# sgl-project/rbg

Hardware: AMD Instinct MI355X
Metric: output tok/s (llama-3-8b P/D-disagg serving, KV migration over xGMI) (higher is better)
Workload: dtype bf16; 1 GPU; model=llama-3-8b, global_batch=128, seq_len=2048, parallelism=pd1 (1 prefill + 1 decode, prefill colocated with decode0)

## Files before the change

rbg_amd/models/llama.py:

```python
from __future__ import annotations

import math
from dataclasses import dataclass
from typing import Optional

import torch
import torch.nn as nn

from .. import ops
from ..engine.config import ModelConfig
from ..engine.kv_cache import PagedKVCache


@dataclass
class ForwardBatch:
    mode: str
    positions: torch.Tensor
    slot_mapping: torch.Tensor
    cu_seqlens: Optional[torch.Tensor] = None
    cu_seqlens_k: Optional[torch.Tensor] = None
    kv_gather_slots: Optional[torch.Tensor] = None
    block_tables: Optional[torch.Tensor] = None
    context_lens: Optional[torch.Tensor] = None
    decode_num_splits: int = 0
# ... 100 lines not shown
        wk = _linear_weight(full_kv, cfg.hidden_size, device, dtype, gen,
                            shard_dim=0, tp_size=tp.size, tp_rank=tp.rank)
        wv = _linear_weight(full_kv, cfg.hidden_size, device, dtype, gen,
                            shard_dim=0, tp_size=tp.size, tp_rank=tp.rank)
        self.wqkv = nn.Parameter(torch.cat([wq, wk, wv], dim=0),
                                 requires_grad=False)
        self.wo = _linear_weight(cfg.hidden_size, full_q, device, dtype, gen,
                                 shard_dim=1, tp_size=tp.size,
                                 tp_rank=tp.rank)
        self.q_out, self.kv_out = q_out, kv_out
        self.q_norm = self.k_norm = None
        if cfg.qk_norm:
            self.q_norm = nn.Parameter(torch.ones(cfg.head_dim, device=device,
                                                  dtype=dtype),
                                       requires_grad=False)
            self.k_norm = nn.Parameter(torch.ones(cfg.head_dim, device=device,
                                                  dtype=dtype),
                                       requires_grad=False)

    def forward(self, x: torch.Tensor, batch: ForwardBatch,
                kv: PagedKVCache, cos_sin: torch.Tensor,
                add_norm=None) -> torch.Tensor:
        T = x.shape[0]
        qkv = ops.linear(x, self.wqkv)
        q = qkv[:, :self.q_out]
        k = qkv[:, self.q_out:self.q_out + self.kv_out]
        v = qkv[:, self.q_out + self.kv_out:]
        if self.q_norm is not None:
            q = ops.rmsnorm(q.contiguous().view(-1, self.head_dim),
                            self.q_norm,
                            self.cfg.rms_eps).view(T, self.q_out)
            k = ops.rmsnorm(k.contiguous().view(-1, self.head_dim),
                            self.k_norm,
                            self.cfg.rms_eps).view(T, self.kv_out)
            v = v.clone(memory_format=torch.contiguous_format)
        key_cache = kv.key_cache(self.layer_idx)
        value_cache = kv.value_cache(self.layer_idx)
        fp8 = kv.fp8
        if fp8:
            ops.rope_store_kv(q, k, v, key_cache, value_cache, cos_sin,
                              batch.positions, batch.slot_mapping,
                              kv.k_scale_log2, kv.v_scale_log2)
        else:
            ops.rope_store_kv(q, k, v, key_cache, value_cache, cos_sin,
                              batch.positions, batch.slot_mapping)
        q3 = q.view(T, self.heads, self.head_dim)
        if batch.mode == "prefill":
            if fp8:
                if batch.kv_gather_slots is None:
                    raise RuntimeError("an fp8 KV pool prefills through the "
                                       "gather path: kv_gather_slots unset")
                k_full = ops.kv_gather_dequant(
                    key_cache, batch.kv_gather_slots, kv.k_scale_log2)
                v_full = ops.kv_gather_dequant(
                    value_cache, batch.kv_gather_slots, kv.v_scale_log2)
                o = ops.prefill_attention(q3, k_full, v_full,
                                          batch.cu_seqlens, self.scale,
                                          batch.cu_seqlens_k)
            elif batch.kv_gather_slots is not None:
                ps = key_cache.shape[2]
                slots = batch.kv_gather_slots.long()
                pages, offs = slots // ps, slots % ps
# ... 190 lines not shown
```

rbg_amd/ops/__init__.py:

```python
from __future__ import annotations

import os

import torch

from . import reference

_hip = None
_hip_err: Exception | None = None
try:
    from . import _hip_ops as _hip
except Exception as e:
    _hip_err = e

HAVE_HIP = _hip is not None


def _check_stale() -> None:
    import hashlib
    here = os.path.dirname(os.path.abspath(__file__))
    stamp = os.path.join(here, "_hip_ops.srchash")
    if not os.path.exists(stamp):
        return
    h = hashlib.sha256()
# ... 26 lines not shown
    return _hip


def _on_gpu(t: torch.Tensor) -> bool:
    return t.is_cuda


SKINNY_GEMM = int(os.environ.get("RBG_SKINNY_GEMM", "1"))


def linear(x: torch.Tensor, w: torch.Tensor) -> torch.Tensor:
    if _use_skinny_gemm(x, w):
        return _require_hip().skinny_gemm(
            x if x.is_contiguous() else x.contiguous(), w)
    return torch.nn.functional.linear(x, w)


def _use_skinny_gemm(x: torch.Tensor, w: torch.Tensor) -> bool:
    return bool(SKINNY_GEMM and _on_gpu(x) and x.dim() == 2 and
                x.dtype == torch.bfloat16 and 1 <= x.shape[0] <= 128 and
                w.shape[0] % 32 == 0 and x.shape[1] % 512 == 0 and
                (w.shape[0] <= 4608 or
                 (x.shape[0] <= 64 and w.shape[0] <= 8192)))


def linear_add_rmsnorm(x: torch.Tensor, w: torch.Tensor,
                       residual: torch.Tensor, norm_weight: torch.Tensor,
                       eps: float) -> torch.Tensor:
    if _use_skinny_gemm(x, w):
        return _require_hip().skinny_gemm_add_rmsnorm(
            x if x.is_contiguous() else x.contiguous(), w, residual,
            norm_weight, eps)
    h = linear(x, w)
    fused_add_rmsnorm(h, residual, norm_weight, eps)
    return h


def rmsnorm(x: torch.Tensor, weight: torch.Tensor, eps: float) -> torch.Tensor:
    if _on_gpu(x):
        return _require_hip().rmsnorm(x, weight, eps)
    return reference.rmsnorm(x, weight, eps)


def fused_add_rmsnorm(x: torch.Tensor, residual: torch.Tensor,
                      weight: torch.Tensor, eps: float) -> None:
    if _on_gpu(x):
# ... 144 lines not shown
```

rbg_amd/ops/hip/bindings.cpp:

```cpp
#include <torch/extension.h>
#include <ATen/hip/HIPContext.h>

#include <hip/hip_runtime.h>

#include <algorithm>
#include <cmath>
#include <cstring>
#include <vector>

extern "C" {
void launch_rmsnorm(void*, void*, const void*, float, int, int, hipStream_t);
void launch_fused_add_rmsnorm(void*, void*, const void*, float, int, int,
                              hipStream_t);
void launch_silu_mul(void*, const void*, int, int, hipStream_t);
void launch_rope_store_kv(void*, void*, const void*, void*, void*,
                          const void*, const void*, const void*, int, int,
                          int, int, int, int, int, hipStream_t);
void launch_decode_attention(void*, void*, void*, const void*, const void*,
                             const void*, const void*, const void*, float,
                             int, int, int, int, int, int, int, int, int,
                             hipStream_t);
void launch_prefill_attention(void*, const void*, const void*, const void*,
                              const void*, const void*, float, int, int, int,
                              int, int, int, hipStream_t);
void launch_mfma_probe(void*, const void*, const void*, int, int, hipStream_t);
void launch_mfma_probe32(void*, const void*, const void*, int, int, int,
                         hipStream_t);
void launch_skinny_gemm(void*, void*, const void*, const void*, int, int,
                        int, int, hipStream_t);
void launch_skinny_gemm_wide(void*, void*, const void*, const void*, int, int,
                             int, int, hipStream_t);
void launch_reduce_splits(void*, const void*, int, long, hipStream_t);
void launch_fold_add_rmsnorm(void*, const void*, void*, const void*, float,
                             int, int, int, hipStream_t);
void launch_kv_peer_copy(void*, const void*, const void*, const void*, int,
                         int, int, long, long, long, long, hipStream_t);
void launch_xgmi_allreduce(void*, const void*, void**, void**, int, int,
                           long, hipStream_t);
void launch_sample(void*, void*, const void*, const void*, const void*,
                   const void*, const void*, const void*, const void*, int,
                   int, hipStream_t);
void launch_rope_store_kv_fp8(void*, void*, const void*, void*, void*,
                              const void*, const void*, const void*, int, int,
                              int, int, int, int, float, float, hipStream_t);
void launch_kv_gather_dequant(void*, const void*, const void*, long, int, int,
                              int, float, hipStream_t);
void launch_decode_attention_fp8(void*, void*, void*, const void*, const void*,
                                 const void*, const void*, const void*, float,
                                 float, int, int, int, int, int, int, int,
                                 hipStream_t);
long xgmi_allreduce_signal_bytes();
long xgmi_allreduce_error_offset();
long xgmi_allreduce_counter_offset();
}
// ... 79 lines not shown
  out_sizes.back() = inter;
  auto out = torch::empty(out_sizes, x.options());
  if (tokens == 0) return out;
  launch_silu_mul(out.data_ptr(), x.data_ptr(), tokens, inter,
                  current_stream());
  return out;
}

static void check_bf16_rowslice(const torch::Tensor& t, const char* name) {
  TORCH_CHECK(t.is_cuda(), name, " must be on GPU");
  TORCH_CHECK(t.scalar_type() == torch::kBFloat16, name, " must be bf16");
  if (t.dim() == 2) {
    TORCH_CHECK(t.stride(1) == 1, name, " rows must be contiguous");
  } else {
    TORCH_CHECK(t.dim() == 3 && t.stride(2) == 1 &&
                t.stride(1) == t.size(2), name,
                " must be [T, H, D] with contiguous (H, D) rows");
  }
}

void rope_store_kv(torch::Tensor q, torch::Tensor k, torch::Tensor v,
                   torch::Tensor key_cache, torch::Tensor value_cache,
                   torch::Tensor cos_sin, torch::Tensor positions,
                   torch::Tensor slot_mapping) {
  check_bf16_rowslice(q, "q");
  check_bf16_rowslice(k, "k");
  check_bf16_rowslice(v, "v");
  TORCH_CHECK(k.stride(0) == v.stride(0), "k/v stride mismatch");
  TORCH_CHECK(cos_sin.scalar_type() == torch::kFloat32, "cos_sin fp32");
  TORCH_CHECK(positions.scalar_type() == torch::kInt32, "positions int32");
  TORCH_CHECK(slot_mapping.scalar_type() == torch::kInt32, "slots int32");
  check_kv_caches(key_cache, value_cache);
  check_i32_gpu(positions, "positions");
  check_i32_gpu(slot_mapping, "slot_mapping");
  TORCH_CHECK(cos_sin.is_cuda() && cos_sin.is_contiguous() &&
              cos_sin.dim() == 2, "cos_sin must be a contiguous 2-D GPU tensor");
  const int tokens = q.size(0);
  const int head_dim = key_cache.size(3);
  const int num_kv_heads = key_cache.size(1);
  const int page_size = key_cache.size(2);
  TORCH_CHECK(cos_sin.size(1) == head_dim,
              "cos_sin row width must equal the cache head_dim");
  TORCH_CHECK(k.size(0) == tokens && v.size(0) == tokens &&
              positions.numel() == tokens && slot_mapping.numel() == tokens,
              "q/k/v/positions/slot_mapping token counts differ");
  const int64_t q_width = q.numel() / std::max(tokens, 1);
  const int64_t k_width = k.numel() / std::max(tokens, 1);
  const int64_t v_width = v.numel() / std::max(tokens, 1);
  TORCH_CHECK(k_width == (int64_t)num_kv_heads * head_dim && v_width == k_width,
              "k/v rows must be cache KVH * head_dim wide");
  TORCH_CHECK(q_width % head_dim == 0,
              "q row width must be a multiple of the cache head_dim");
  if (tokens == 0) return;
  const int num_q_heads = (int)(q_width / head_dim);
  launch_rope_store_kv(q.data_ptr(), k.data_ptr(), v.data_ptr(),
                       key_cache.data_ptr(), value_cache.data_ptr(),
                       cos_sin.data_ptr(), positions.data_ptr(),
                       slot_mapping.data_ptr(), tokens, num_q_heads,
                       num_kv_heads, head_dim, page_size,
                       (int)q.stride(0), (int)k.stride(0),
                       current_stream());
}

bool pick_in_wg_combine(int64_t combine, int64_t num_splits, bool mfma_pair,
                        const char* what) {
  TORCH_CHECK(combine >= 0 && combine <= 2,
              "combine must be 0 (auto), 1 (kernel) or 2 (in-workgroup)");
  const bool can = mfma_pair && (num_splits == 2 || num_splits == 4);
  TORCH_CHECK(combine != 2 || can, "combine = 2 needs ", what,
              ", a page size of 16 and 2 or 4 splits");
  const bool in_wg = combine != 1 && can;
  TORCH_CHECK(!in_wg || num_splits == 2 || num_splits == 4,
              "in-workgroup combine with ", num_splits, " splits");
  return in_wg;
}

torch::Tensor decode_attention(torch::Tensor q, torch::Tensor key_cache,
                               torch::Tensor value_cache,
                               torch::Tensor block_tables,
                               torch::Tensor context_lens, double scale,
                               int64_t num_splits, int64_t variant,
                               int64_t combine = 0) {
  TORCH_CHECK(q.is_cuda() && q.scalar_type() == torch::kBFloat16 &&
              q.dim() == 3 && q.stride(2) == 1 &&
// ... 240 lines not shown
  return d;
}

}

static int pick_gemm_splits(int N, int K) {
  const int n_groups = N >> 5;
  for (int s : {8, 4, 2})
    if (n_groups * s <= 512 && n_groups * s >= 192 && K % (s * 256) == 0)
      return s;
  for (int s : {4, 2})
    if (n_groups * s >= 128 && K % (s * 256) == 0) return s;
  return 1;
}

bool skinny_gemm_supported(int64_t M, int64_t N, int64_t K) {
  return M >= 1 && M <= 256 && (N % 32) == 0 && (K % 256) == 0;
}

bool skinny_gemm_wide_supported(int64_t M, int64_t N) {
  return M >= 1 && M <= 128 && (N % 64) == 0;
}

static int pick_gemm_panel(int64_t M, int64_t N) {
  return M > 32 && skinny_gemm_wide_supported(M, N) ? 64 : 32;
}

namespace {

int skinny_gemm_launch(const torch::Tensor& a, const torch::Tensor& w,
                       int64_t force_splits, int64_t panel, torch::Tensor& c,
                       torch::Tensor& ws) {
  check_bf16_contig(a, "a");
  check_bf16_contig(w, "w");
  TORCH_CHECK(a.dim() == 2 && w.dim() == 2, "a and w must be 2-D");
  TORCH_CHECK(a.device() == w.device(), "a/w device mismatch");
  const int64_t M = a.size(0), K = a.size(1), N = w.size(0);
  TORCH_CHECK(w.size(1) == K, "K mismatch");
  TORCH_CHECK(skinny_gemm_supported(M, N, K), "unsupported skinny shape");
  TORCH_CHECK(force_splits == 0 || force_splits == 1 || force_splits == 2 ||
                  force_splits == 4 || force_splits == 8,
              "force_splits must be 0 (auto), 1, 2, 4 or 8");
  TORCH_CHECK(force_splits == 0 || K % (force_splits * 256) == 0,
              "K must be a multiple of force_splits * 256");
  TORCH_CHECK(panel == 0 || panel == 32 || panel == 64,
              "panel must be 0 (auto), 32 or 64");
  TORCH_CHECK(panel != 64 || skinny_gemm_wide_supported(M, N),
              "panel 64 needs M <= 128 and N % 64 == 0");
  const int splits = force_splits > 0 ? (int)force_splits
                                      : pick_gemm_splits((int)N, (int)K);
  if (panel == 0) panel = pick_gemm_panel(M, N);
  void* cp = nullptr;
  void* wsp = nullptr;
  if (splits > 1) {
    ws = torch::empty({splits, M, N}, a.options().dtype(torch::kFloat32));
    wsp = ws.data_ptr();
  } else {
    c = torch::empty({M, N}, a.options());
    cp = c.data_ptr();
  }
  (panel == 64 ? launch_skinny_gemm_wide : launch_skinny_gemm)(
      cp, wsp, a.data_ptr(), w.data_ptr(), (int)M, (int)N, (int)K, splits,
      current_stream());
  return splits;
}

}

torch::Tensor skinny_gemm(torch::Tensor a, torch::Tensor w,
                          int64_t force_splits = 0, int64_t panel = 0) {
  torch::Tensor c, ws;
  const int splits = skinny_gemm_launch(a, w, force_splits, panel, c, ws);
  if (splits > 1) {
    c = torch::empty({a.size(0), w.size(0)}, a.options());
    launch_reduce_splits(c.data_ptr(), ws.data_ptr(), splits,
                         (long)c.numel(), current_stream());
  }
  return c;
}

torch::Tensor skinny_gemm_add_rmsnorm(torch::Tensor a, torch::Tensor w,
                                      torch::Tensor residual,
                                      torch::Tensor norm_weight, double eps,
                                      int64_t force_splits = 0,
                                      int64_t panel = 0) {
  check_bf16_contig(residual, "residual");
  check_bf16_contig(norm_weight, "norm_weight");
  TORCH_CHECK(a.dim() == 2 && w.dim() == 2, "a and w must be 2-D");
  TORCH_CHECK(residual.dim() == 2 && residual.size(0) == a.size(0) &&
                  residual.size(1) == w.size(0),
              "residual must be [M, N]");
  TORCH_CHECK(norm_weight.numel() == w.size(0),
              "norm_weight must have N elements");
  TORCH_CHECK(residual.device() == a.device() &&
                  norm_weight.device() == a.device(),
              "a/residual/norm_weight device mismatch");
  torch::Tensor c, ws;
  const int splits = skinny_gemm_launch(a, w, force_splits, panel, c, ws);
  const int M = (int)a.size(0), N = (int)w.size(0);
  if (splits == 1) {
    launch_fused_add_rmsnorm(c.data_ptr(), residual.data_ptr(),
                             norm_weight.data_ptr(), (float)eps, M, N,
                             current_stream());
    return c;
  }
  c = torch::empty({a.size(0), w.size(0)}, a.options());
  launch_fold_add_rmsnorm(c.data_ptr(), ws.data_ptr(), residual.data_ptr(),
                          norm_weight.data_ptr(), (float)eps, splits, M, N,
                          current_stream());
  return c;
}


std::vector<torch::Tensor> sample(torch::Tensor logits,
                                  torch::Tensor temperature,
                                  torch::Tensor top_k, torch::Tensor top_p,
                                  torch::Tensor min_p, torch::Tensor seed,
                                  torch::Tensor pos) {
  TORCH_CHECK(logits.is_cuda(), "logits must be on GPU");
  TORCH_CHECK(logits.scalar_type() == torch::kFloat32, "logits must be fp32");
  TORCH_CHECK(logits.dim() == 2, "logits must be [n, V]");
  TORCH_CHECK(logits.is_contiguous(), "logits must be contiguous");
  const int64_t n = logits.size(0), V = logits.size(1);
  TORCH_CHECK(V >= 1, "V must be >= 1");
  TORCH_CHECK(V <= INT32_MAX && n <= INT32_MAX, "n and V must fit int32");
  auto check_param = [&](const torch::Tensor& t, torch::ScalarType dt,
                         const char* name) {
    TORCH_CHECK(t.is_cuda() && t.device() == logits.device(), name,
                " must be on the logits' device");
    TORCH_CHECK(t.scalar_type() == dt, name, " has the wrong dtype");
    TORCH_CHECK(t.dim() == 1 && t.size(0) == n, name,
                " must have one entry per row");
// ... 150 lines not shown
  check_bf16_contig(inp, "inp");
  const int world = (int)sig_ptrs.size();
  TORCH_CHECK(world >= 1 && world <= 8 &&
                  data_ptrs.size() == (size_t)world && rank >= 0 &&
                  rank < world,
              "bad world/rank");
  TORCH_CHECK(inp.numel() % 8 == 0, "numel must be a multiple of 8");
  auto out = torch::empty_like(inp);
  void* sp[8];
  void* dp[8];
  for (int i = 0; i < world; ++i) {
    sp[i] = reinterpret_cast<void*>(sig_ptrs[i]);
    dp[i] = reinterpret_cast<void*>(data_ptrs[i]);
  }
  launch_xgmi_allreduce(out.data_ptr(), inp.data_ptr(), sp, dp, world,
                        (int)rank, (long)inp.numel(), current_stream());
  return out;
}

PYBIND11_MODULE(TORCH_EXTENSION_NAME, m) {
  m.def("rmsnorm", &rmsnorm, "RMSNorm (bf16)");
  m.def("fused_add_rmsnorm", &fused_add_rmsnorm, "x,residual += ; rmsnorm");
  m.def("silu_mul", &silu_mul, "silu(gate)*up");
  m.def("rope_store_kv", &rope_store_kv, "RoPE + paged KV write");
  m.def("decode_attention", &decode_attention, "paged flash-decode",
        py::arg("q"), py::arg("key_cache"), py::arg("value_cache"),
        py::arg("block_tables"), py::arg("context_lens"), py::arg("scale"),
        py::arg("num_splits"), py::arg("variant"), py::arg("combine") = 0);
  m.def("rope_store_kv_fp8", &rope_store_kv_fp8,
        "RoPE + quantising (e4m3) paged KV write");
  m.def("kv_gather_dequant", &kv_gather_dequant,
        "gather e4m3 cache rows by slot -> bf16 [Tkv, KVH, D]");
  m.def("decode_attention_fp8", &decode_attention_fp8,
        "paged flash-decode over an e4m3 cache (page-pair MFMA)",
        py::arg("q"), py::arg("key_cache"), py::arg("value_cache"),
        py::arg("block_tables"), py::arg("context_lens"), py::arg("scale"),
        py::arg("num_splits"), py::arg("k_scale_log2"),
        py::arg("v_scale_log2"), py::arg("combine") = 0);
  m.def("prefill_attention", &prefill_attention, "varlen causal flash prefill");
  m.def("mfma_probe", &mfma_probe, "MFMA layout probe");
  m.def("mfma_probe32", &mfma_probe32, "32x32x16 MFMA layout probe");
  m.def("skinny_gemm", &skinny_gemm, "decode-shape GEMM (M<=128)",
        py::arg("a"), py::arg("w"), py::arg("force_splits") = 0,
        py::arg("panel") = 0);
  m.def("skinny_gemm_add_rmsnorm", &skinny_gemm_add_rmsnorm,
        "skinny_gemm + fused_add_rmsnorm with the split-K fold inside the "
        "norm kernel; returns h, updates residual in place",
        py::arg("a"), py::arg("w"), py::arg("residual"),
        py::arg("norm_weight"), py::arg("eps"), py::arg("force_splits") = 0,
        py::arg("panel") = 0);
  m.def("sample", &sample,
        "seeded top-k/min-p/top-p Gumbel-max sampler -> (tokens, num_kept)");
  m.def("ipc_alloc_bf16", &ipc_alloc_bf16,
        "hipMalloc-backed bf16 tensor (IPC-exportable base allocation)",
        py::call_guard<py::gil_scoped_release>());
  m.def("ipc_alloc", &ipc_alloc,
        "hipMalloc-backed tensor of any dtype (IPC-exportable allocation)",
        py::call_guard<py::gil_scoped_release>());
  m.def("kv_ipc_export", &kv_ipc_export, "hipIpcGetMemHandle of a KV pool");
  m.def("kv_ipc_open", &kv_ipc_open,
        "map a peer KV pool (lazy xGMI peer access)",
        py::call_guard<py::gil_scoped_release>());
  m.def("kv_ipc_close", &kv_ipc_close, "unmap a peer KV pool",
        py::call_guard<py::gil_scoped_release>());
  m.def("kv_peer_copy", &kv_peer_copy,
        "gather local pages -> scatter into peer pool over xGMI",
        py::call_guard<py::gil_scoped_release>());
  m.def("ar_alloc_signals", &ar_alloc_signals,
        "uncached signal buffer for the xGMI all-reduce");
  m.def("ar_export_ptr", &ar_export_ptr, "hipIpc handle of a raw pointer");
  m.def("ar_error_flag", &ar_error_flag, "read the all-reduce error word");
  m.def("ar_dump_signals", &ar_dump_signals, "debug: dump the signal block");
  m.def("ar_counter_offset", &xgmi_allreduce_counter_offset);
// ... 4 lines not shown
```

rbg_amd/ops/hip/rope_kv.hip:

```cpp
#include "common.h"

namespace {

__global__ void rope_store_kv_kernel(
    __hip_bfloat16* __restrict__ q,
    __hip_bfloat16* __restrict__ k,
    const __hip_bfloat16* __restrict__ v,
    __hip_bfloat16* __restrict__ key_cache,
    __hip_bfloat16* __restrict__ val_cache,
    const float* __restrict__ cos_sin,
    const int* __restrict__ positions,
    const int* __restrict__ slot_mapping,
    const int num_q_heads, const int num_kv_heads, const int head_dim,
    const int page_size,
    const int q_stride, const int kv_stride) {
  const int token = blockIdx.x;
  const int tid = threadIdx.x;
  const int pos = positions[token];
  const int slot = slot_mapping[token];
  const int half = head_dim / 2;
  const float* cs = cos_sin + (size_t)pos * head_dim;

  __hip_bfloat16* q_tok = q + (size_t)token * q_stride;
  const int q_pairs = num_q_heads * half;
// ... 20 lines not shown
    const __hip_bfloat16 r2 = f2bf(x2 * c + x1 * s);
    base[d] = r1;
    base[d + half] = r2;
    if (slot >= 0) {
      __hip_bfloat16* kdst = key_cache +
          (((size_t)page * num_kv_heads + h) * page_size + poff) * head_dim;
      kdst[d] = r1;
      kdst[d + half] = r2;
    }
  }
  if (slot >= 0) {
    const int nvec = num_kv_heads * head_dim / 8;
    for (int i = tid; i < nvec; i += blockDim.x) {
      const int h = (i * 8) / head_dim;
      const int d = (i * 8) % head_dim;
      __hip_bfloat16* vdst = val_cache +
          (((size_t)page * num_kv_heads + h) * page_size + poff) * head_dim;
      *reinterpret_cast<uint4*>(vdst + d) =
          *reinterpret_cast<const uint4*>(v_tok + h * head_dim + d);
    }
  }
}

}

extern "C" {

void launch_rope_store_kv(void* q, void* k, const void* v, void* key_cache,
                          void* val_cache, const void* cos_sin,
                          const void* positions, const void* slot_mapping,
                          int tokens, int num_q_heads, int num_kv_heads,
                          int head_dim, int page_size, int q_stride,
                          int kv_stride, hipStream_t stream) {
  dim3 grid(tokens), block(256);
  hipLaunchKernelGGL(rope_store_kv_kernel, grid, block, 0, stream,
                     (__hip_bfloat16*)q, (__hip_bfloat16*)k,
                     (const __hip_bfloat16*)v, (__hip_bfloat16*)key_cache,
                     (__hip_bfloat16*)val_cache, (const float*)cos_sin,
                     (const int*)positions, (const int*)slot_mapping,
                     num_q_heads, num_kv_heads, head_dim, page_size,
                     q_stride, kv_stride);
}

}
```

rbg_amd/ops/hip/skinny_gemm.hip:

```cpp
#include "common.h"

typedef __attribute__((ext_vector_type(8))) __bf16 gg_bf8;

DEV_INLINE gg_bf8 lds_frag(const __hip_bfloat16* p) {
  union { uint4 u; gg_bf8 v; } cvt;
  cvt.u = *reinterpret_cast<const uint4*>(p);
  return cvt.v;
}

#define SG_KSTEP 64
#define SG_LDS_PITCH (SG_KSTEP + 8)
#define SG_NT 256

template <int M_TILES, int SPLITS>
__global__ __launch_bounds__(SG_NT, 3) void skinny_gemm_kernel(
    const __hip_bfloat16* __restrict__ a,
    const __hip_bfloat16* __restrict__ w,
    __hip_bfloat16* __restrict__ c,
    float* __restrict__ ws,
    const int M, const int N, const int K) {
  const int n_groups = N >> 5;
  const int n_group = blockIdx.x % n_groups;
  const int split = blockIdx.x / n_groups;
  const int tid = threadIdx.x;
// ... 283 lines not shown
#pragma unroll
    for (int mt = 0; mt < MTW; ++mt)
#pragma unroll
      for (int nt = 0; nt < 4; ++nt) {
        F32x4U u;
        u.v = acc[mt][nt];
        const int n = (n_group << 6) + (nt << 4) + gl;
#pragma unroll
        for (int r = 0; r < 4; ++r) {
          const float v =
              u.e[r] + lds.red[row_group][(mt * 4 + nt) * 256 + r * 64 + lane];
          const int m = (row_group * MTW + mt) * 16 + (gslice << 2) + r;
          if (m < M) {
            if (SPLITS == 1)
              c[(size_t)m * N + n] = f2bf(v);
            else
              ws[((size_t)split * M + m) * N + n] = v;
          }
        }
      }
  }
}

__global__ void reduce_splits_kernel(const float* __restrict__ ws,
                                     __hip_bfloat16* __restrict__ c,
                                     const int splits, const long mn) {
  const long i = (long)blockIdx.x * blockDim.x + threadIdx.x;
  if (i >= mn) return;
  float v = 0.f;
  for (int s = 0; s < splits; ++s) v += ws[(size_t)s * mn + i];
  c[i] = f2bf(v);
}


extern "C" void launch_skinny_gemm(void* c, void* ws, const void* a,
                                   const void* w, int M, int N, int K,
                                   int splits, hipStream_t stream) {
  const dim3 grid((N >> 5) * splits), block(SG_NT);
  const __hip_bfloat16* ap = (const __hip_bfloat16*)a;
  const __hip_bfloat16* wp = (const __hip_bfloat16*)w;
  __hip_bfloat16* cp = (__hip_bfloat16*)c;
  float* wsp = (float*)ws;
  const int m_tiles = (M + 15) >> 4;

#define LAUNCH_MT(MT)                                                        \
  do {                                                                       \
// ... 29 lines not shown
  float* wsp = (float*)ws;

#define LAUNCH_MTW(MTW)                                                      \
  do {                                                                       \
    if (splits == 1)                                                         \
      skinny_gemm_wide_kernel<MTW, 1><<<grid, block, 0, stream>>>(           \
          ap, wp, cp, nullptr, M, N, K);                                     \
    else if (splits == 2)                                                    \
      skinny_gemm_wide_kernel<MTW, 2><<<grid, block, 0, stream>>>(           \
          ap, wp, cp, wsp, M, N, K);                                         \
    else if (splits == 4)                                                    \
      skinny_gemm_wide_kernel<MTW, 4><<<grid, block, 0, stream>>>(           \
          ap, wp, cp, wsp, M, N, K);                                         \
    else                                                                     \
      skinny_gemm_wide_kernel<MTW, 8><<<grid, block, 0, stream>>>(           \
          ap, wp, cp, wsp, M, N, K);                                         \
  } while (0)

  if (M <= 64) LAUNCH_MTW(1);
  else LAUNCH_MTW(2);
#undef LAUNCH_MTW
}

extern "C" void launch_reduce_splits(void* c, const void* ws, int splits,
                                     long mn, hipStream_t stream) {
  const int threads = 256;
  reduce_splits_kernel<<<dim3((mn + threads - 1) / threads), dim3(threads),
                         0, stream>>>((const float*)ws, (__hip_bfloat16*)c,
                                      splits, mn);
}
```

Before: 11050 tok/s.

## Fuse QKV GEMM with RoPE/KV store, add LDS-DMA GEMM and vectorized RoPE

Adds a fused QKV projection path that folds the split-K partials inside the RoPE/KV-store kernel. This removes the separate reduce_splits launch and a round trip of the qkv tensor. It also adds a new skinny GEMM variant that loads A and W tiles straight into LDS through global_load_lds with a 4-deep ring, used by default for M in 16..64. A 16-byte vectorized rope_store_kv kernel is also added. Together these add a lot of hand-written asm and pipelining code, which raises correctness and tuning risk.

After: 11130 tok/s (median of 6 runs). About the same (+0.7%).

```diff
diff --git a/rbg_amd/models/llama.py b/rbg_amd/models/llama.py
--- a/rbg_amd/models/llama.py
+++ b/rbg_amd/models/llama.py
@@ -146,7 +146,18 @@
                 kv: PagedKVCache, cos_sin: torch.Tensor,
                 add_norm=None) -> torch.Tensor:
         T = x.shape[0]
-        qkv = ops.linear(x, self.wqkv)
+        key_cache = kv.key_cache(self.layer_idx)
+        value_cache = kv.value_cache(self.layer_idx)
+        fp8 = kv.fp8
+        fused_rope = (self.q_norm is None and not fp8 and
+                      ops._use_skinny_gemm(x, self.wqkv))
+        if fused_rope:
+            qkv = ops.linear_rope_store_kv(
+                x, self.wqkv, key_cache, value_cache, cos_sin,
+                batch.positions, batch.slot_mapping, self.heads,
+                self.kv_heads, self.head_dim)
+        else:
+            qkv = ops.linear(x, self.wqkv)
         q = qkv[:, :self.q_out]
         k = qkv[:, self.q_out:self.q_out + self.kv_out]
         v = qkv[:, self.q_out + self.kv_out:]
@@ -158,10 +169,9 @@
                             self.k_norm,
                             self.cfg.rms_eps).view(T, self.kv_out)
             v = v.clone(memory_format=torch.contiguous_format)
-        key_cache = kv.key_cache(self.layer_idx)
-        value_cache = kv.value_cache(self.layer_idx)
-        fp8 = kv.fp8
-        if fp8:
+        if fused_rope:
+            pass
+        elif fp8:
             ops.rope_store_kv(q, k, v, key_cache, value_cache, cos_sin,
                               batch.positions, batch.slot_mapping,
                               kv.k_scale_log2, kv.v_scale_log2)
diff --git a/rbg_amd/ops/__init__.py b/rbg_amd/ops/__init__.py
--- a/rbg_amd/ops/__init__.py
+++ b/rbg_amd/ops/__init__.py
@@ -72,6 +72,25 @@
                 w.shape[0] % 32 == 0 and x.shape[1] % 512 == 0 and
                 (w.shape[0] <= 4608 or
                  (x.shape[0] <= 64 and w.shape[0] <= 8192)))
+
+
+def linear_rope_store_kv(x: torch.Tensor, wqkv: torch.Tensor, key_cache,
+                         value_cache, cos_sin, positions, slot_mapping,
+                         num_q_heads: int, num_kv_heads: int,
+                         head_dim: int) -> torch.Tensor:
+    if _is_fp8_pair(key_cache, value_cache):
+        raise ValueError("linear_rope_store_kv writes a bf16 KV cache only")
+    if _use_skinny_gemm(x, wqkv) and head_dim % 16 == 0:
+        return _require_hip().skinny_gemm_rope_store_kv(
+            x if x.is_contiguous() else x.contiguous(), wqkv, key_cache,
+            value_cache, cos_sin, positions, slot_mapping, num_q_heads,
+            num_kv_heads, head_dim)
+    qkv = linear(x, wqkv)
+    q_out, kv_out = num_q_heads * head_dim, num_kv_heads * head_dim
+    rope_store_kv(qkv[:, :q_out], qkv[:, q_out:q_out + kv_out],
+                  qkv[:, q_out + kv_out:], key_cache, value_cache, cos_sin,
+                  positions, slot_mapping)
+    return qkv
 
 
 def linear_add_rmsnorm(x: torch.Tensor, w: torch.Tensor,
diff --git a/rbg_amd/ops/hip/bindings.cpp b/rbg_amd/ops/hip/bindings.cpp
--- a/rbg_amd/ops/hip/bindings.cpp
+++ b/rbg_amd/ops/hip/bindings.cpp
@@ -15,7 +15,10 @@
 void launch_silu_mul(void*, const void*, int, int, hipStream_t);
 void launch_rope_store_kv(void*, void*, const void*, void*, void*,
                           const void*, const void*, const void*, int, int,
-                          int, int, int, int, int, hipStream_t);
+                          int, int, int, int, int, int, hipStream_t);
+void launch_rope_store_kv_fold(const void*, void*, void*, void*, const void*,
+                               const void*, const void*, int, int, int, int,
+                               int, int, hipStream_t);
 void launch_decode_attention(void*, void*, void*, const void*, const void*,
                              const void*, const void*, const void*, float,
                              int, int, int, int, int, int, int, int, int,
@@ -30,6 +33,8 @@
                         int, int, hipStream_t);
 void launch_skinny_gemm_wide(void*, void*, const void*, const void*, int, int,
                              int, int, hipStream_t);
+void launch_skinny_gemm_wide_dma(void*, void*, const void*, const void*, int,
+                                 int, int, int, hipStream_t);
 void launch_reduce_splits(void*, const void*, int, long, hipStream_t);
 void launch_fold_add_rmsnorm(void*, const void*, void*, const void*, float,
                              int, int, int, hipStream_t);
@@ -155,7 +160,7 @@
 void rope_store_kv(torch::Tensor q, torch::Tensor k, torch::Tensor v,
                    torch::Tensor key_cache, torch::Tensor value_cache,
                    torch::Tensor cos_sin, torch::Tensor positions,
-                   torch::Tensor slot_mapping) {
+                   torch::Tensor slot_mapping, int64_t vec = 0) {
   check_bf16_rowslice(q, "q");
   check_bf16_rowslice(k, "k");
   check_bf16_rowslice(v, "v");
@@ -186,13 +191,23 @@
               "q row width must be a multiple of the cache head_dim");
   if (tokens == 0) return;
   const int num_q_heads = (int)(q_width / head_dim);
+  TORCH_CHECK(vec >= 0 && vec <= 2,
+              "vec must be 0 (auto), 1 (element-wise) or 2 (16-byte)");
+  auto aligned = [](const torch::Tensor& t) {
+    return reinterpret_cast<uintptr_t>(t.data_ptr()) % 16 == 0 &&
+           t.stride(0) % 8 == 0;
+  };
+  const bool can_vec = head_dim % 16 == 0 && aligned(q) && aligned(k) &&
+                       aligned(v);
+  TORCH_CHECK(vec != 2 || can_vec,
+              "vec 2 needs head_dim % 16 == 0 and 16-byte aligned q/k/v rows");
   launch_rope_store_kv(q.data_ptr(), k.data_ptr(), v.data_ptr(),
                        key_cache.data_ptr(), value_cache.data_ptr(),
                        cos_sin.data_ptr(), positions.data_ptr(),
                        slot_mapping.data_ptr(), tokens, num_q_heads,
                        num_kv_heads, head_dim, page_size,
                        (int)q.stride(0), (int)k.stride(0),
-                       current_stream());
+                       vec == 1 ? 0 : (int)can_vec, current_stream());
 }
 
 bool pick_in_wg_combine(int64_t combine, int64_t num_splits, bool mfma_pair,
@@ -479,15 +494,24 @@
   return M >= 1 && M <= 128 && (N % 64) == 0;
 }
 
+static bool pick_gemm_dma(int64_t M, int64_t N) {
+  return M >= 16 && M <= 64 && skinny_gemm_wide_supported(M, N);
+}
+
 static int pick_gemm_panel(int64_t M, int64_t N) {
-  return M > 32 && skinny_gemm_wide_supported(M, N) ? 64 : 32;
+  return (M > 32 || pick_gemm_dma(M, N)) && skinny_gemm_wide_supported(M, N)
+             ? 64 : 32;
+}
+
+static int pick_gemm_stage(int64_t M, int64_t N, int64_t panel) {
+  return panel == 64 && pick_gemm_dma(M, N) ? 2 : 1;
 }
 
 namespace {
 
 int skinny_gemm_launch(const torch::Tensor& a, const torch::Tensor& w,
-                       int64_t force_splits, int64_t panel, torch::Tensor& c,
-                       torch::Tensor& ws) {
+                       int64_t force_splits, int64_t panel, int64_t stage,
+                       torch::Tensor& c, torch::Tensor& ws) {
   check_bf16_contig(a, "a");
   check_bf16_contig(w, "w");
   TORCH_CHECK(a.dim() == 2 && w.dim() == 2, "a and w must be 2-D");
@@ -504,9 +528,16 @@
               "panel must be 0 (auto), 32 or 64");
   TORCH_CHECK(panel != 64 || skinny_gemm_wide_supported(M, N),
               "panel 64 needs M <= 128 and N % 64 == 0");
+  TORCH_CHECK(stage >= 0 && stage <= 2,
+              "stage must be 0 (auto), 1 (registers) or 2 (LDS-DMA)");
+  TORCH_CHECK(stage < 2 || (panel != 32 && skinny_gemm_wide_supported(M, N)),
+              "stage 2 (LDS-DMA) needs the 64-column panel: M <= 128 and "
+              "N % 64 == 0");
   const int splits = force_splits > 0 ? (int)force_splits
                                       : pick_gemm_splits((int)N, (int)K);
-  if (panel == 0) panel = pick_gemm_panel(M, N);
+  if (panel == 0)
+    panel = stage == 2 ? 64 : stage == 1 && M <= 32 ? 32 : pick_gemm_panel(M, N);
+  if (stage == 0) stage = pick_gemm_stage(M, N, panel);
   void* cp = nullptr;
   void* wsp = nullptr;
   if (splits > 1) {
@@ -516,18 +547,24 @@
     c = torch::empty({M, N}, a.options());
     cp = c.data_ptr();
   }
-  (panel == 64 ? launch_skinny_gemm_wide : launch_skinny_gemm)(
-      cp, wsp, a.data_ptr(), w.data_ptr(), (int)M, (int)N, (int)K, splits,
-      current_stream());
+  if (stage == 2)
+    launch_skinny_gemm_wide_dma(cp, wsp, a.data_ptr(), w.data_ptr(), (int)M,
+                                (int)N, (int)K, splits, current_stream());
+  else
+    (panel == 64 ? launch_skinny_gemm_wide : launch_skinny_gemm)(
+        cp, wsp, a.data_ptr(), w.data_ptr(), (int)M, (int)N, (int)K, splits,
+        current_stream());
   return splits;
 }
 
 }
 
 torch::Tensor skinny_gemm(torch::Tensor a, torch::Tensor w,
-                          int64_t force_splits = 0, int64_t panel = 0) {
+                          int64_t force_splits = 0, int64_t panel = 0,
+                          int64_t stage = 0) {
   torch::Tensor c, ws;
-  const int splits = skinny_gemm_launch(a, w, force_splits, panel, c, ws);
+  const int splits =
+      skinny_gemm_launch(a, w, force_splits, panel, stage, c, ws);
   if (splits > 1) {
     c = torch::empty({a.size(0), w.size(0)}, a.options());
     launch_reduce_splits(c.data_ptr(), ws.data_ptr(), splits,
@@ -536,11 +573,21 @@
   return c;
 }
 
+torch::Tensor skinny_gemm_partials(torch::Tensor a, torch::Tensor w,
+                                   int64_t force_splits = 0,
+                                   int64_t panel = 0, int64_t stage = 0) {
+  torch::Tensor c, ws;
+  const int splits =
+      skinny_gemm_launch(a, w, force_splits, panel, stage, c, ws);
+  TORCH_CHECK(splits > 1, "a launch with one split has no partials");
+  return ws;
+}
+
 torch::Tensor skinny_gemm_add_rmsnorm(torch::Tensor a, torch::Tensor w,
                                       torch::Tensor residual,
                                       torch::Tensor norm_weight, double eps,
                                       int64_t force_splits = 0,
-                                      int64_t panel = 0) {
+                                      int64_t panel = 0, int64_t stage = 0) {
   check_bf16_contig(residual, "residual");
   check_bf16_contig(norm_weight, "norm_weight");
   TORCH_CHECK(a.dim() == 2 && w.dim() == 2, "a and w must be 2-D");
@@ -553,7 +600,8 @@
                   norm_weight.device() == a.device(),
               "a/residual/norm_weight device mismatch");
   torch::Tensor c, ws;
-  const int splits = skinny_gemm_launch(a, w, force_splits, panel, c, ws);
+  const int splits =
+      skinny_gemm_launch(a, w, force_splits, panel, stage, c, ws);
   const int M = (int)a.size(0), N = (int)w.size(0);
   if (splits == 1) {
     launch_fused_add_rmsnorm(c.data_ptr(), residual.data_ptr(),
@@ -565,6 +613,57 @@
   launch_fold_add_rmsnorm(c.data_ptr(), ws.data_ptr(), residual.data_ptr(),
                           norm_weight.data_ptr(), (float)eps, splits, M, N,
                           current_stream());
+  return c;
+}
+
+torch::Tensor skinny_gemm_rope_store_kv(
+    torch::Tensor x, torch::Tensor wqkv, torch::Tensor key_cache,
+    torch::Tensor value_cache, torch::Tensor cos_sin, torch::Tensor positions,
+    torch::Tensor slot_mapping, int64_t num_q_heads, int64_t num_kv_heads,
+    int64_t head_dim, int64_t force_splits = 0, int64_t panel = 0,
+    int64_t stage = 0) {
+  TORCH_CHECK(x.dim() == 2 && wqkv.dim() == 2, "x and wqkv must be 2-D");
+  const int64_t T = x.size(0), N = wqkv.size(0);
+  TORCH_CHECK(num_q_heads > 0 && num_kv_heads > 0 && head_dim > 0 &&
+                  N == (num_q_heads + 2 * num_kv_heads) * head_dim,
+              "wqkv must have (num_q_heads + 2 * num_kv_heads) * head_dim rows");
+  TORCH_CHECK(head_dim % 16 == 0, "head_dim must be a multiple of 16");
+  check_kv_caches(key_cache, value_cache);
+  TORCH_CHECK(key_cache.size(1) == num_kv_heads &&
+                  key_cache.size(3) == head_dim,
+              "cache KVH / head_dim differ from the projection's");
+  check_i32_gpu(positions, "positions");
+  check_i32_gpu(slot_mapping, "slot_mapping");
+  TORCH_CHECK(positions.numel() == T && slot_mapping.numel() == T,
+              "x/positions/slot_mapping token counts differ");
+  TORCH_CHECK(cos_sin.is_cuda() && cos_sin.is_contiguous() &&
+                  cos_sin.dim() == 2 &&
+                  cos_sin.scalar_type() == torch::kFloat32 &&
+                  cos_sin.size(1) == head_dim,
+              "cos_sin must be a contiguous fp32 [max_pos, head_dim] GPU tensor");
+  TORCH_CHECK(key_cache.device() == x.device() &&
+                  cos_sin.device() == x.device() &&
+                  positions.device() == x.device() &&
+                  slot_mapping.device() == x.device(),
+              "x/cache/cos_sin/positions/slot_mapping device mismatch");
+  torch::Tensor c, ws;
+  const int splits =
+      skinny_gemm_launch(x, wqkv, force_splits, panel, stage, c, ws);
+  if (splits == 1) {
+    const int64_t q_out = num_q_heads * head_dim;
+    const int64_t kv_out = num_kv_heads * head_dim;
+    rope_store_kv(c.slice(1, 0, q_out), c.slice(1, q_out, q_out + kv_out),
+                  c.slice(1, q_out + kv_out, N), key_cache, value_cache,
+                  cos_sin, positions, slot_mapping);
+    return c;
+  }
+  c = torch::empty({T, N}, x.options());
+  launch_rope_store_kv_fold(ws.data_ptr(), c.data_ptr(), key_cache.data_ptr(),
+                            value_cache.data_ptr(), cos_sin.data_ptr(),
+                            positions.data_ptr(), slot_mapping.data_ptr(),
+                            splits, (int)T, (int)num_q_heads,
+                            (int)num_kv_heads, (int)head_dim,
+                            (int)key_cache.size(2), current_stream());
   return c;
 }
 
@@ -761,7 +860,10 @@
   m.def("rmsnorm", &rmsnorm, "RMSNorm (bf16)");
   m.def("fused_add_rmsnorm", &fused_add_rmsnorm, "x,residual += ; rmsnorm");
   m.def("silu_mul", &silu_mul, "silu(gate)*up");
-  m.def("rope_store_kv", &rope_store_kv, "RoPE + paged KV write");
+  m.def("rope_store_kv", &rope_store_kv, "RoPE + paged KV write",
+        py::arg("q"), py::arg("k"), py::arg("v"), py::arg("key_cache"),
+        py::arg("value_cache"), py::arg("cos_sin"), py::arg("positions"),
+        py::arg("slot_mapping"), py::arg("vec") = 0);
   m.def("decode_attention", &decode_attention, "paged flash-decode",
         py::arg("q"), py::arg("key_cache"), py::arg("value_cache"),
         py::arg("block_tables"), py::arg("context_lens"), py::arg("scale"),
@@ -781,13 +883,26 @@
   m.def("mfma_probe32", &mfma_probe32, "32x32x16 MFMA layout probe");
   m.def("skinny_gemm", &skinny_gemm, "decode-shape GEMM (M<=128)",
         py::arg("a"), py::arg("w"), py::arg("force_splits") = 0,
-        py::arg("panel") = 0);
+        py::arg("panel") = 0, py::arg("stage") = 0);
+  m.def("skinny_gemm_partials", &skinny_gemm_partials,
+        "the f32 split-K partials [splits, M, N] of skinny_gemm, unfolded",
+        py::arg("a"), py::arg("w"), py::arg("force_splits") = 0,
+        py::arg("panel") = 0, py::arg("stage") = 0);
   m.def("skinny_gemm_add_rmsnorm", &skinny_gemm_add_rmsnorm,
         "skinny_gemm + fused_add_rmsnorm with the split-K fold inside the "
         "norm kernel; returns h, updates residual in place",
         py::arg("a"), py::arg("w"), py::arg("residual"),
         py::arg("norm_weight"), py::arg("eps"), py::arg("force_splits") = 0,
-        py::arg("panel") = 0);
+        py::arg("panel") = 0, py::arg("stage") = 0);
+  m.def("skinny_gemm_rope_store_kv", &skinny_gemm_rope_store_kv,
+        "skinny_gemm + rope_store_kv with the split-K fold inside the RoPE "
+        "kernel; returns the post-RoPE qkv",
+        py::arg("x"), py::arg("wqkv"), py::arg("key_cache"),
+        py::arg("value_cache"), py::arg("cos_sin"), py::arg("positions"),
+        py::arg("slot_mapping"), py::arg("num_q_heads"),
+        py::arg("num_kv_heads"), py::arg("head_dim"),
+        py::arg("force_splits") = 0, py::arg("panel") = 0,
+        py::arg("stage") = 0);
   m.def("sample", &sample,
         "seeded top-k/min-p/top-p Gumbel-max sampler -> (tokens, num_kept)");
   m.def("ipc_alloc_bf16", &ipc_alloc_bf16,
diff --git a/rbg_amd/ops/hip/rope_kv.hip b/rbg_amd/ops/hip/rope_kv.hip
--- a/rbg_amd/ops/hip/rope_kv.hip
+++ b/rbg_amd/ops/hip/rope_kv.hip
@@ -66,16 +66,213 @@
   }
 }
 
+DEV_INLINE void fold8(const float* __restrict__ p, const size_t mn,
+                      const int splits, float* v) {
+#pragma unroll
+  for (int j = 0; j < 8; ++j) v[j] = 0.f;
+  for (int s = 0; s < splits; ++s) {
+    const float4 lo = *reinterpret_cast<const float4*>(p + (size_t)s * mn);
+    const float4 hi = *reinterpret_cast<const float4*>(p + (size_t)s * mn + 4);
+    v[0] += lo.x; v[1] += lo.y; v[2] += lo.z; v[3] += lo.w;
+    v[4] += hi.x; v[5] += hi.y; v[6] += hi.z; v[7] += hi.w;
+  }
+}
+
+DEV_INLINE void rotate8(const float* x1, const float* x2,
+                        const float* __restrict__ cs, const int d,
+                        const int half, Bf16x8U& o1, Bf16x8U& o2) {
+  float c[8], s[8];
+  *reinterpret_cast<float4*>(c) = *reinterpret_cast<const float4*>(cs + d);
+  *reinterpret_cast<float4*>(c + 4) =
+      *reinterpret_cast<const float4*>(cs + d + 4);
+  *reinterpret_cast<float4*>(s) =
+      *reinterpret_cast<const float4*>(cs + half + d);
+  *reinterpret_cast<float4*>(s + 4) =
+      *reinterpret_cast<const float4*>(cs + half + d + 4);
+#pragma unroll
+  for (int j = 0; j < 8; ++j) {
+    o1.e[j] = f2bf(x1[j] * c[j] - x2[j] * s[j]);
+    o2.e[j] = f2bf(x2[j] * c[j] + x1[j] * s[j]);
+  }
+}
+
+__global__ __launch_bounds__(256) void rope_store_kv_vec_kernel(
+    __hip_bfloat16* __restrict__ q, __hip_bfloat16* __restrict__ k,
+    const __hip_bfloat16* __restrict__ v,
+    __hip_bfloat16* __restrict__ key_cache,
+    __hip_bfloat16* __restrict__ val_cache, const float* __restrict__ cos_sin,
+    const int* __restrict__ positions, const int* __restrict__ slot_mapping,
+    const int num_q_heads, const int num_kv_heads, const int head_dim,
+    const int page_size, const int q_stride, const int kv_stride,
+    const int parts) {
+  const int token = blockIdx.x / parts;
+  const int part = blockIdx.x - token * parts;
+  const int pos = positions[token];
+  const int slot = slot_mapping[token];
+  const int half = head_dim >> 1;
+  const int hv = half >> 3;
+  const float* cs = cos_sin + (size_t)pos * head_dim;
+  __hip_bfloat16* q_tok = q + (size_t)token * q_stride;
+  __hip_bfloat16* k_tok = k + (size_t)token * kv_stride;
+  const __hip_bfloat16* v_tok = v + (size_t)token * kv_stride;
+  const int page = slot >= 0 ? slot / page_size : 0;
+  const int poff = slot >= 0 ? slot % page_size : 0;
+  const int rot_items = (num_q_heads + num_kv_heads) * hv;
+  const int v_items = slot >= 0 ? num_kv_heads * (head_dim >> 3) : 0;
+
+  for (int i = part * blockDim.x + threadIdx.x; i < rot_items + v_items;
+       i += parts * blockDim.x) {
+    if (i < rot_items) {
+      const int h = i / hv, d = (i - h * hv) << 3;
+      const bool is_k = h >= num_q_heads;
+      __hip_bfloat16* base = is_k ? k_tok + (h - num_q_heads) * head_dim
+                                  : q_tok + h * head_dim;
+      Bf16x8U i1, i2, o1, o2;
+      i1.u = *reinterpret_cast<const uint4*>(base + d);
+      i2.u = *reinterpret_cast<const uint4*>(base + d + half);
+      float a1[8], a2[8];
+#pragma unroll
+      for (int j = 0; j < 8; ++j) {
+        a1[j] = bf2f(i1.e[j]);
+        a2[j] = bf2f(i2.e[j]);
+      }
+      rotate8(a1, a2, cs, d, half, o1, o2);
+      *reinterpret_cast<uint4*>(base + d) = o1.u;
+      *reinterpret_cast<uint4*>(base + d + half) = o2.u;
+      if (is_k && slot >= 0) {
+        __hip_bfloat16* kdst = key_cache +
+            (((size_t)page * num_kv_heads + (h - num_q_heads)) * page_size +
+             poff) * head_dim;
+        *reinterpret_cast<uint4*>(kdst + d) = o1.u;
+        *reinterpret_cast<uint4*>(kdst + d + half) = o2.u;
+      }
+    } else {
+      const int e = (i - rot_items) << 3;
+      const int h = e / head_dim, d = e - h * head_dim;
+      __hip_bfloat16* vdst = val_cache +
+          (((size_t)page * num_kv_heads + h) * page_size + poff) * head_dim;
+      *reinterpret_cast<uint4*>(vdst + d) =
+          *reinterpret_cast<const uint4*>(v_tok + e);
+    }
+  }
+}
+
+__global__ __launch_bounds__(256) void rope_store_kv_fold_kernel(
+    const float* __restrict__ ws,
+    __hip_bfloat16* __restrict__ qkv,
+    __hip_bfloat16* __restrict__ key_cache,
+    __hip_bfloat16* __restrict__ val_cache,
+    const float* __restrict__ cos_sin,
+    const int* __restrict__ positions,
+    const int* __restrict__ slot_mapping,
+    const int splits, const int tokens, const int num_q_heads,
+    const int num_kv_heads, const int head_dim, const int page_size,
+    const int parts) {
+  const int token = blockIdx.x / parts;
+  const int part = blockIdx.x - token * parts;
+  const int pos = positions[token];
+  const int slot = slot_mapping[token];
+  const int half = head_dim >> 1;
+  const int hv = half >> 3;
+  const int N = (num_q_heads + 2 * num_kv_heads) * head_dim;
+  const size_t mn = (size_t)tokens * N;
+  const float* cs = cos_sin + (size_t)pos * head_dim;
+  const float* ws_tok = ws + (size_t)token * N;
+  __hip_bfloat16* out_tok = qkv + (size_t)token * N;
+  const int page = slot >= 0 ? slot / page_size : 0;
+  const int poff = slot >= 0 ? slot % page_size : 0;
+  const int rot_items = (num_q_heads + num_kv_heads) * hv;
+  const int v_items = num_kv_heads * (head_dim >> 3);
+  const int v_col0 = (num_q_heads + num_kv_heads) * head_dim;
+
+  for (int i = part * blockDim.x + threadIdx.x; i < rot_items + v_items;
+       i += parts * blockDim.x) {
+    if (i < rot_items) {
+      const int h = i / hv, d = (i - h * hv) << 3;
+      const int col = h * head_dim + d;
+      float a1[8], a2[8];
+      fold8(ws_tok + col, mn, splits, a1);
+      fold8(ws_tok + col + half, mn, splits, a2);
+#pragma unroll
+      for (int j = 0; j < 8; ++j) {
+        a1[j] = bf2f(f2bf(a1[j]));
+        a2[j] = bf2f(f2bf(a2[j]));
+      }
+      Bf16x8U o1, o2;
+      rotate8(a1, a2, cs, d, half, o1, o2);
+      *reinterpret_cast<uint4*>(out_tok + col) = o1.u;
+      *reinterpret_cast<uint4*>(out_tok + col + half) = o2.u;
+      if (h >= num_q_heads && slot >= 0) {
+        __hip_bfloat16* kdst = key_cache +
+            (((size_t)page * num_kv_heads + (h - num_q_heads)) * page_size +
+             poff) * head_dim;
+        *reinterpret_cast<uint4*>(kdst + d) = o1.u;
+        *reinterpret_cast<uint4*>(kdst + d + half) = o2.u;
+      }
+    } else {
+      const int e = (i - rot_items) << 3;
+      const int h = e / head_dim, d = e - h * head_dim;
+      float a[8];
+      fold8(ws_tok + v_col0 + e, mn, splits, a);
+      Bf16x8U o;
+#pragma unroll
+      for (int j = 0; j < 8; ++j) o.e[j] = f2bf(a[j]);
+      *reinterpret_cast<uint4*>(out_tok + v_col0 + e) = o.u;
+      if (slot >= 0) {
+        __hip_bfloat16* vdst = val_cache +
+            (((size_t)page * num_kv_heads + h) * page_size + poff) * head_dim;
+        *reinterpret_cast<uint4*>(vdst + d) = o.u;
+      }
+    }
+  }
+}
+
+int rope_parts(int tokens, int items) {
+  return (tokens < 256 && items > 256) ? 2 : 1;
+}
+
 }
 
 extern "C" {
+
+void launch_rope_store_kv_fold(const void* ws, void* qkv, void* key_cache,
+                               void* val_cache, const void* cos_sin,
+                               const void* positions,
+                               const void* slot_mapping, int splits,
+                               int tokens, int num_q_heads, int num_kv_heads,
+                               int head_dim, int page_size,
+                               hipStream_t stream) {
+  const int items = (num_q_heads + num_kv_heads) * (head_dim >> 4) +
+                    num_kv_heads * (head_dim >> 3);
+  const int parts = rope_parts(tokens, items);
+  dim3 grid(tokens * parts), block(256);
+  hipLaunchKernelGGL(rope_store_kv_fold_kernel, grid, block, 0, stream,
+                     (const float*)ws, (__hip_bfloat16*)qkv,
+                     (__hip_bfloat16*)key_cache, (__hip_bfloat16*)val_cache,
+                     (const float*)cos_sin, (const int*)positions,
+                     (const int*)slot_mapping, splits, tokens, num_q_heads,
+                     num_kv_heads, head_dim, page_size, parts);
+}
 
 void launch_rope_store_kv(void* q, void* k, const void* v, void* key_cache,
                           void* val_cache, const void* cos_sin,
                           const void* positions, const void* slot_mapping,
                           int tokens, int num_q_heads, int num_kv_heads,
                           int head_dim, int page_size, int q_stride,
-                          int kv_stride, hipStream_t stream) {
+                          int kv_stride, int vec, hipStream_t stream) {
+  if (vec) {
+    const int items = (num_q_heads + num_kv_heads) * (head_dim >> 4) +
+                      num_kv_heads * (head_dim >> 3);
+    const int parts = rope_parts(tokens, items);
+    hipLaunchKernelGGL(rope_store_kv_vec_kernel, dim3(tokens * parts),
+                       dim3(256), 0, stream, (__hip_bfloat16*)q,
+                       (__hip_bfloat16*)k, (const __hip_bfloat16*)v,
+                       (__hip_bfloat16*)key_cache, (__hip_bfloat16*)val_cache,
+                       (const float*)cos_sin, (const int*)positions,
+                       (const int*)slot_mapping, num_q_heads, num_kv_heads,
+                       head_dim, page_size, q_stride, kv_stride, parts);
+    return;
+  }
   dim3 grid(tokens), block(256);
   hipLaunchKernelGGL(rope_store_kv_kernel, grid, block, 0, stream,
                      (__hip_bfloat16*)q, (__hip_bfloat16*)k,
diff --git a/rbg_amd/ops/hip/skinny_gemm.hip b/rbg_amd/ops/hip/skinny_gemm.hip
--- a/rbg_amd/ops/hip/skinny_gemm.hip
+++ b/rbg_amd/ops/hip/skinny_gemm.hip
@@ -329,6 +329,157 @@
   }
 }
 
+#define SGD_ROW_BYTES 128
+#define SGD_DEPTH 4
+
+DEV_INLINE void sgd_glds16(const void* gsrc, const unsigned lds_dst) {
+  unsigned keep;
+  asm volatile(
+      "s_mov_b32 %0, m0\n\t"
+      "s_mov_b32 m0, %2\n\t"
+      "s_nop 0\n\t"
+      "global_load_lds_dwordx4 %1, off\n\t"
+      "s_mov_b32 m0, %0"
+      : "=&s"(keep)
+      : "v"(gsrc), "s"(lds_dst)
+      : "memory");
+}
+
+template <int MTW, int SPLITS, int DEPTH>
+__global__ __launch_bounds__(SGW_NT) void skinny_gemm_wide_dma_kernel(
+    const __hip_bfloat16* __restrict__ a,
+    const __hip_bfloat16* __restrict__ w,
+    __hip_bfloat16* __restrict__ c,
+    float* __restrict__ ws,
+    const int M, const int N, const int K) {
+  const int n_groups = N >> 6;
+  const int n_group = blockIdx.x % n_groups;
+  const int split = blockIdx.x / n_groups;
+  const int tid = threadIdx.x;
+  const int wave = __builtin_amdgcn_readfirstlane(tid >> 6);
+  const int lane = tid & 63;
+  const int gl = lane & 15;
+  const int gslice = lane >> 4;
+
+  const int row_group = wave & 3;
+  const int k_slice = wave >> 2;
+  const int k_wg = K / SPLITS;
+  const int k0 = split * k_wg;
+  const int nsteps = k_wg / SG_KSTEP;
+
+  constexpr int A_ROWS = MTW * 64;
+  constexpr int SLOT = (64 + A_ROWS) * SGD_ROW_BYTES;
+  constexpr int PIECES = 1 + MTW;
+  static_assert(DEPTH >= 3 && PIECES * (DEPTH - 2) <= 63, "vmcnt range");
+  __shared__ union {
+    unsigned char ring[DEPTH * SLOT];
+    float red[4][MTW * 4 * 256];
+  } lds;
+  static_assert(sizeof(float) * 4 * MTW * 4 * 256 <= DEPTH * SLOT, "red fits");
+  const unsigned ring_lds = (unsigned)(uintptr_t)(
+      __attribute__((address_space(3))) unsigned char*)lds.ring;
+
+  const int prow = (wave << 3) + (lane >> 3);
+  const int pchk = ((lane & 7) ^ (lane >> 3)) << 3;
+  const __hip_bfloat16* wsrc =
+      w + (size_t)((n_group << 6) + prow) * K + pchk;
+  const __hip_bfloat16* asrc0 = a + (size_t)min(prow, M - 1) * K + pchk;
+  const __hip_bfloat16* asrc1 = a + (size_t)min(prow + 64, M - 1) * K + pchk;
+  const unsigned wave_dst = ring_lds + (wave << 10);
+
+  auto issue = [&](const int tile, const int slot) {
+    const int kb = k0 + min(tile, nsteps - 1) * SG_KSTEP;
+    const unsigned dst = wave_dst + slot * SLOT;
+    sgd_glds16(asrc0 + kb, dst + 64 * SGD_ROW_BYTES);
+    if (MTW > 1) sgd_glds16(asrc1 + kb, dst + 128 * SGD_ROW_BYTES);
+    sgd_glds16(wsrc + kb, dst);
+  };
+
+  f32x4 acc[MTW][4];
+#pragma unroll
+  for (int mt = 0; mt < MTW; ++mt)
+#pragma unroll
+    for (int nt = 0; nt < 4; ++nt) acc[mt][nt] = {0.f, 0.f, 0.f, 0.f};
+
+  const int frag_off = gl * SGD_ROW_BYTES +
+                       ((((k_slice << 2) + gslice) ^ (gl & 7)) << 4);
+  auto frag = [&](const unsigned char* st, const int row0) {
+    union { uint4 u; gg_bf8 v; } cvt;
+    cvt.u = *reinterpret_cast<const uint4*>(st + row0 * SGD_ROW_BYTES +
+                                            frag_off);
+    return cvt.v;
+  };
+  auto compute = [&](const unsigned char* st) {
+    const gg_bf8 wf0 = frag(st, 0);
+    const gg_bf8 wf1 = frag(st, 16);
+    const gg_bf8 wf2 = frag(st, 32);
+    const gg_bf8 wf3 = frag(st, 48);
+#pragma unroll
+    for (int mt = 0; mt < MTW; ++mt) {
+      const gg_bf8 af = frag(st, 64 + (row_group * MTW + mt) * 16);
+      acc[mt][0] = __builtin_amdgcn_mfma_f32_16x16x32_bf16(af, wf0,
+                                                           acc[mt][0], 0, 0, 0);
+      acc[mt][1] = __builtin_amdgcn_mfma_f32_16x16x32_bf16(af, wf1,
+                                                           acc[mt][1], 0, 0, 0);
+      acc[mt][2] = __builtin_amdgcn_mfma_f32_16x16x32_bf16(af, wf2,
+                                                           acc[mt][2], 0, 0, 0);
+      acc[mt][3] = __builtin_amdgcn_mfma_f32_16x16x32_bf16(af, wf3,
+                                                           acc[mt][3], 0, 0, 0);
+    }
+  };
+
+#pragma unroll
+  for (int t = 0; t < DEPTH - 1; ++t) issue(t, t);
+
+  int slot = 0;
+  for (int step = 0; step < nsteps; ++step) {
+    asm volatile("s_waitcnt vmcnt(%0) lgkmcnt(0)"
+                 :: "n"(PIECES * (DEPTH - 2)) : "memory");
+    __builtin_amdgcn_s_barrier();
+    issue(step + DEPTH - 1, slot == 0 ? DEPTH - 1 : slot - 1);
+    compute(lds.ring + slot * SLOT);
+    slot = slot + 1 == DEPTH ? 0 : slot + 1;
+  }
+
+  asm volatile("s_waitcnt vmcnt(0) lgkmcnt(0)" ::: "memory");
+  __syncthreads();
+  if (k_slice == 1) {
+#pragma unroll
+    for (int mt = 0; mt < MTW; ++mt)
+#pragma unroll
+      for (int nt = 0; nt < 4; ++nt) {
+        F32x4U u;
+        u.v = acc[mt][nt];
+#pragma unroll
+        for (int r = 0; r < 4; ++r)
+          lds.red[row_group][(mt * 4 + nt) * 256 + r * 64 + lane] = u.e[r];
+      }
+  }
+  __syncthreads();
+  if (k_slice == 0) {
+#pragma unroll
+    for (int mt = 0; mt < MTW; ++mt)
+#pragma unroll
+      for (int nt = 0; nt < 4; ++nt) {
+        F32x4U u;
+        u.v = acc[mt][nt];
+        const int n = (n_group << 6) + (nt << 4) + gl;
+#pragma unroll
+        for (int r = 0; r < 4; ++r) {
+          const float v =
+              u.e[r] + lds.red[row_group][(mt * 4 + nt) * 256 + r * 64 + lane];
+          const int m = (row_group * MTW + mt) * 16 + (gslice << 2) + r;
+          if (m < M) {
+            if (SPLITS == 1)
+              c[(size_t)m * N + n] = f2bf(v);
+            else
+              ws[((size_t)split * M + m) * N + n] = v;
+          }
+        }
+      }
+  }
+}
+
 __global__ void reduce_splits_kernel(const float* __restrict__ ws,
                                      __hip_bfloat16* __restrict__ c,
                                      const int splits, const long mn) {
@@ -404,6 +555,36 @@
 #undef LAUNCH_MTW
 }
 
+extern "C" void launch_skinny_gemm_wide_dma(void* c, void* ws, const void* a,
+                                            const void* w, int M, int N, int K,
+                                            int splits, hipStream_t stream) {
+  const dim3 grid((N >> 6) * splits), block(SGW_NT);
+  const __hip_bfloat16* ap = (const __hip_bfloat16*)a;
+  const __hip_bfloat16* wp = (const __hip_bfloat16*)w;
+  __hip_bfloat16* cp = (__hip_bfloat16*)c;
+  float* wsp = (float*)ws;
+
+#define LAUNCH_DMA(MTW)                                                      \
+  do {                                                                       \
+    if (splits == 1)                                                         \
+      skinny_gemm_wide_dma_kernel<MTW, 1, SGD_DEPTH>                         \
+          <<<grid, block, 0, stream>>>(ap, wp, cp, nullptr, M, N, K);        \
+    else if (splits == 2)                                                    \
+      skinny_gemm_wide_dma_kernel<MTW, 2, SGD_DEPTH>                         \
+          <<<grid, block, 0, stream>>>(ap, wp, cp, wsp, M, N, K);            \
+    else if (splits == 4)                                                    \
+      skinny_gemm_wide_dma_kernel<MTW, 4, SGD_DEPTH>                         \
+          <<<grid, block, 0, stream>>>(ap, wp, cp, wsp, M, N, K);            \
+    else                                                                     \
+      skinny_gemm_wide_dma_kernel<MTW, 8, SGD_DEPTH>                         \
+          <<<grid, block, 0, stream>>>(ap, wp, cp, wsp, M, N, K);            \
+  } while (0)
+
+  if (M <= 64) LAUNCH_DMA(1);
+  else LAUNCH_DMA(2);
+#undef LAUNCH_DMA
+}
+
 extern "C" void launch_reduce_splits(void* c, const void* ws, int splits,
                                      long mn, hipStream_t stream) {
   const int threads = 256;
```
